# naver/deep-image-retrieval

Measured on AMD Instinct MI355X. Metric: images/sec descriptor extraction (resnet101-GeM, 1024x1024), higher is better.
Workload: dtype fp16p

## Files before the change

deep-image-retrieval_amd/csrc/conv_igemm.h:

```cpp
#pragma once
#include "dir_common.h"

namespace dir {

struct ConvArgs {
    const uint16_t* x;
    const uint16_t* w;
    const float* bias;
    const uint16_t* res;
    uint16_t* y;
    int B, H, W, Cin, OH, OW, Cout;
    int R, S, stride, pad, relu;
    int M;
    int Ktot;
    int T;
    int ksplit;
    float* partial;
    const uint16_t* w2;
    const float* bias2;
    uint16_t* y2;
    int Cout2, relu2;
    const uint16_t* x2;
    int Cin2;
    int H2, W2, stride2;
// ... 70 lines not shown
    a.T = a.Ktot / 64;
}
inline void conv_args_second_source(ConvArgs& a, const uint16_t* x2, const uint16_t* x2_lo, int Cin2) {
    a.x2 = x2;
    a.x2_lo = x2_lo;
    a.Cin2 = Cin2;
    a.Ktot = a.Cin + Cin2;
    a.T = a.Ktot / 64;
}
inline void conv_args_next_conv1(ConvArgs& a, const uint16_t* w2, const uint16_t* w2_lo, const float* bias2, uint16_t* y2,
                                 int Cout2, int relu2) {
    a.w2 = w2;
    a.w2_lo = w2_lo;
    a.bias2 = bias2;
    a.y2 = y2;
    a.Cout2 = Cout2;
    a.relu2 = relu2;
}

typedef bool (*ConvAdmissibleFn)(const ConvArgs&);
typedef hipError_t (*ConvLaunchFn)(const ConvArgs&, int dtype, hipStream_t);

struct ConvVariant {
    const char* name;
    int BM, BN, threads, stages, BK;
    ConvAdmissibleFn admissible;
    ConvLaunchFn launch;
    bool has_splitk;
    ConvAdmissibleFn admissible_dual;
    ConvLaunchFn launch_dual;
};

bool conv1x1_persist_admissible(const ConvArgs& a);
hipError_t conv1x1_persist_launch(const ConvArgs& a, int dtype, hipStream_t stream);
bool conv1x1_persist_x3_admissible(const ConvArgs& a);
hipError_t conv1x1_persist_x3_launch(const ConvArgs& a, int dtype, hipStream_t stream);
bool conv1x1_persist_dual_admissible(const ConvArgs& a);
hipError_t conv1x1_persist_dual_launch(const ConvArgs& a, int dtype, hipStream_t stream);
bool conv_patch64_lc_admissible(const ConvArgs& a);
hipError_t conv_patch64_lc_launch(const ConvArgs& a, int dtype, hipStream_t stream);
bool conv1x1_ring_admissible(const ConvArgs& a);
hipError_t conv1x1_ring_launch(const ConvArgs& a, int dtype, hipStream_t stream);
bool conv1x1_wreg_admissible(const ConvArgs& a);
hipError_t conv1x1_wreg_launch(const ConvArgs& a, int dtype, hipStream_t stream);
bool conv_small_admissible(const ConvArgs& a);
bool conv_small_k2_admissible(const ConvArgs& a);
hipError_t conv_small_s8_launch(const ConvArgs& a, int dtype, hipStream_t stream);
hipError_t conv_small_s4_launch(const ConvArgs& a, int dtype, hipStream_t stream);
hipError_t conv_small_s4k2_launch(const ConvArgs& a, int dtype, hipStream_t stream);
bool conv1x1_lc_admissible(const ConvArgs& a);
bool conv1x1_lc_plain_admissible(const ConvArgs& a);
hipError_t conv1x1_lc_launch(const ConvArgs& a, int dtype, hipStream_t stream);
hipError_t conv1x1_lc_dual_launch(const ConvArgs& a, int dtype, hipStream_t stream);
bool conv1x1_wregd_admissible(const ConvArgs& a);
hipError_t conv1x1_wregd_launch(const ConvArgs& a, int dtype, hipStream_t stream);
bool conv_seam3_admissible(const ConvArgs& a);
hipError_t conv_seam3_launch(const ConvArgs& a, int dtype, hipStream_t stream);
bool conv_c3c1_admissible(const ConvArgs& a);
bool conv_c3c1ds_lc_admissible(const ConvArgs& a);
hipError_t conv_c3c1ds_lc_launch(const ConvArgs& a, int dtype, hipStream_t stream);
hipError_t conv_c3c1_launch(const ConvArgs& a, int dtype, hipStream_t stream);
bool conv_patch3x3s_admissible(const ConvArgs& a);
hipError_t conv_patch3x3s_launch(const ConvArgs& a, int dtype, hipStream_t stream);
bool conv_patch3x3w_admissible(const ConvArgs& a);
hipError_t conv_patch3x3w_launch(const ConvArgs& a, int dtype, hipStream_t stream);
hipError_t conv_patch3x3w_pack(const uint16_t* w, uint16_t* out, int Cout, int Cin, hipStream_t stream);
bool conv_patch3x3s2_admissible(const ConvArgs& a);
hipError_t conv_patch3x3s2_launch(const ConvArgs& a, int dtype, hipStream_t stream);
hipError_t conv_patch3x3s2_pack(const uint16_t* w, uint16_t* out, int Cout, int Cin, hipStream_t stream);
bool conv_patch3x3_admissible(const ConvArgs& a);
hipError_t conv_patch3x3_launch(const ConvArgs& a, int dtype, hipStream_t stream);

int conv_pair_launch(const ConvArgs& a, hipStream_t stream);
const char* conv_pair_variant_name(const ConvArgs& a);

int conv_variant_count();
const ConvVariant& conv_variant(int i);
bool conv_variant_admissible(int v, const ConvArgs& a);
int conv_pick_variant(const ConvArgs& a);
int conv_pick_dual_variant(const ConvArgs& a, bool any_size = false);
int conv_launch(const ConvArgs& a, int dtype, int variant, hipStream_t stream);
int conv_splitk_factor(int v, const ConvArgs& a);
size_t conv_splitk_bytes(const ConvArgs& a, int ksplit);
constexpr size_t kSplitKMaxBytes = 64u << 20;
int conv_launch_naive(const ConvArgs& a, int dtype, hipStream_t stream);


}
```

deep-image-retrieval_amd/csrc/conv_persist.hip:

```cpp
#include "dir_common.h"
#include "conv_device.h"
#include "conv_igemm.h"

namespace dir {

template <class DT, bool XDEEP, bool RES, bool DUAL = false>
__global__ void __launch_bounds__(512) conv1x1_persist_kernel(const ConvArgs a) {
    static_assert(!DUAL || (XDEEP && !RES), "the two-source form rides on the deep-X ring");
    constexpr int BM = 256, BN = 256, NT = 512;
    constexpr int TM = 2, TN = 4;
    constexpr int NA = 4, NB = 4;
    constexpr int XS = BM * 128, STAGE = (BM + BN) * 128;
    constexpr int EROW = Staged<2>::EROW;
    constexpr int EPI_OFF = XDEEP ? XS : STAGE;
    constexpr int WOFF = 3 * XS;
    typedef typename DT::frag_t frag_t;

    extern __shared__ __attribute__((aligned(16))) char smem[];

    const int tid = threadIdx.x;
    const int lane = tid & 63;
    const int wave = __builtin_amdgcn_readfirstlane(tid >> 6);
    const int wn = wave & 1, wm = wave >> 1;
    const int lrow = lane & 31, lhi = lane >> 5;
    const int srcchunk = (tid & 7) ^ ((tid >> 4) & 7);

    const __amdgpu_buffer_rsrc_t rsrc_x = buffer_rsrc(a.x, a.x_bytes);
    const __amdgpu_buffer_rsrc_t rsrc_w = buffer_rsrc(a.w, a.w_bytes);
    const __amdgpu_buffer_rsrc_t rsrc_x2 = buffer_rsrc(DUAL ? a.x2 : a.x, DUAL ? a.x2_bytes : a.x_bytes);

    const int ntiles = a.tiles_m * a.tiles_n;
    const int T = a.T;
    const int T1 = DUAL ? a.Cin / 64 : 0;

    uint32_t xvoff[NA], wvoff[NB], xvoff2[DUAL ? NA : 1];
    auto tile_offsets = [&](int tile) {
        const int tile_n = tile % a.tiles_n, tile_m = a.rev_m ? a.tiles_m - 1 - tile / a.tiles_n : tile / a.tiles_n;
#pragma unroll
        for (int i = 0; i < NA; ++i) {
            const int m = tile_m * BM + i * 64 + (tid >> 3);
            uint32_t off;
            if (a.flat) {
#ifdef DIR_PERSIST_BLOCKED
                off = (uint32_t)(tile_m * (BM * a.Cin * 2) + (i * 64 + (tid >> 3)) * 128 + srcchunk * 16);
#else
                off = (uint32_t)((m * a.Cin + srcchunk * 8) * 2);
#endif
            } else {
                const uint32_t mm = m < a.M ? (uint32_t)m : 0u;
                const uint32_t b = fast_div(mm, a.div_ohw_mul, a.div_ohw_shr);
                const uint32_t rem = mm - b * (uint32_t)(a.OH * a.OW);
                const uint32_t oh = fast_div(rem, a.div_ow_mul, a.div_ow_shr);
                const uint32_t ow = rem - oh * (uint32_t)a.OW;
                off = (uint32_t)((((b * a.H + oh * a.stride) * a.W + ow * a.stride) * a.Cin +
                                  srcchunk * 8) * 2);
            }
            xvoff[i] = m < a.M ? off : kOOB;
            if (DUAL) {
                const uint32_t mm = m < a.M ? (uint32_t)m : 0u;
                const uint32_t b = fast_div(mm, a.div_ohw_mul, a.div_ohw_shr);
                const uint32_t rem = mm - b * (uint32_t)(a.OH * a.OW);
                const uint32_t oh = fast_div(rem, a.div_ow_mul, a.div_ow_shr);
                const uint32_t ow = rem - oh * (uint32_t)a.OW;
                const uint32_t off2 = (uint32_t)((((b * a.H2 + oh * a.stride2) * a.W2 + ow * a.stride2) * a.Cin2 +
                                                  srcchunk * 8) * 2);
                xvoff2[DUAL ? i : 0] = m < a.M ? off2 : kOOB;
            }
        }
#pragma unroll
        for (int i = 0; i < NB; ++i)
            wvoff[i] = (uint32_t)(((tile_n * BN + i * 64 + (tid >> 3)) * a.Ktot + srcchunk * 8) * 2);
    };
    auto issue_x = [&](int t, char* dst) {
        if (DUAL && t >= T1) {
#pragma unroll
            for (int i = 0; i < NA; ++i)
                dma16(rsrc_x2, dst + (i * NT + wave * 64) * 16, xvoff2[DUAL ? i : 0], (t - T1) * 128);
            return;
        }
#pragma unroll
#ifdef DIR_PERSIST_BLOCKED
        for (int i = 0; i < NA; ++i) dma16(rsrc_x, dst + (i * NT + wave * 64) * 16, xvoff[i], a.flat ? t * (BM * 128) : t * 128);
#else
        for (int i = 0; i < NA; ++i) dma16(rsrc_x, dst + (i * NT + wave * 64) * 16, xvoff[i], t * 128);
#endif
    };
    auto issue_w = [&](int t, char* dst) {
#pragma unroll
        for (int i = 0; i < NB; ++i) dma16(rsrc_w, dst + (i * NT + wave * 64) * 16, wvoff[i], t * 128);
    };
    auto issue = [&](int t, char* stage) {
        issue_x(t, stage);
        issue_w(t, stage + XS);
    };
    auto xslot = [&](int t) { return smem + (t % 3) * XS; };
    auto wslot = [&](int t) { return smem + WOFF + ((t + 1) & 1) * XS; };

    const int lswz = (lane >> 1) & 7;
    int loff[4];
#pragma unroll
    for (int ks = 0; ks < 4; ++ks) loff[ks] = lrow * 128 + (((2 * ks + lhi) ^ lswz) << 4);
    const int xfrag = (wm * TM * 32) * 128;
    const int wfrag = (XDEEP ? 0 : XS) + (wn * TN * 32) * 128;

    int tile = a.no_xcd_map ? (int)blockIdx.x : xcd_remap(blockIdx.x, gridDim.x);
    if (tile >= ntiles) return;
    Ovf<DT> ovf;
    f32x4_t bz[XDEEP ? TN : 1][XDEEP ? 4 : 1];
    auto load_bias = [&](int t) {
        if (!XDEEP) return;
        const int nw = (t % a.tiles_n) * BN + wn * TN * 32;
#pragma unroll
        for (int i = 0; i < TN; ++i)
#pragma unroll
            for (int g = 0; g < 4; ++g)
                bz[XDEEP ? i : 0][XDEEP ? g : 0] = bias4(a.bias + nw + i * 32, g, lhi);
    };
    load_bias(tile);
    tile_offsets(tile);
    if (XDEEP) {
        issue_w(0, wslot(0));
        issue_x(0, xslot(0));
        if (T > 1) issue_x(1, xslot(1));
    } else {
        issue(0, smem);
    }

    for (;;) {
        const int tile_n = tile % a.tiles_n, tile_m = a.rev_m ? a.tiles_m - 1 - tile / a.tiles_n : tile / a.tiles_n;
        const int m_epi = tile_m * BM + wm * TM * 32;
        const int n_wave = tile_n * BN + wn * TN * 32;

        f32x16_t acc[TN][TM];
        acc_init(acc, [&](int i, int g) {
            return XDEEP ? bz[XDEEP ? i : 0][XDEEP ? g : 0] : bias4(a.bias + n_wave + i * 32, g, lhi);
        });

        const int ecol = (lane & 7) * 8, erow = lane >> 3;
        u32x4_t rres[RES ? TM : 1][2][RES ? 4 : 1];
        if (RES && a.res) {
#pragma unroll
            for (int j = 0; j < TM; ++j)
#pragma unroll
                for (int h = 0; h < 2; ++h)
#pragma unroll
                    for (int pass = 0; pass < 4; ++pass) {
                        const int m = m_epi + j * 32 + pass * 8 + erow;
                        const int mc = m < a.M ? m : 0;
                        rres[RES ? j : 0][h][RES ? pass : 0] = gload16(a.res + ((size_t)mc * a.Cout + n_wave + h * 64 + ecol));
                    }
        }

        if (XDEEP) {
            for (int t = 0; t < T; ++t) {
                if (t + 1 < T && !(RES && t == 0 && a.res)) {
                    asm volatile("s_waitcnt vmcnt(%0)" ::"i"(NA) : "memory");
                } else {
                    asm volatile("s_waitcnt vmcnt(0)" ::: "memory");
                }
                ring_barrier();
                if (t + 1 < T) issue_w(t + 1, wslot(t + 1));
                if (t + 2 < T) issue_x(t + 2, xslot(t + 2));
                const char* xs = xslot(t);
                const char* ws = wslot(t);
#pragma unroll
                for (int ks = 0; ks < 4; ++ks) {
                    frag_t wf[TN], xf[TM];
#pragma unroll
                    for (int i = 0; i < TN; ++i) wf[i] = *(const frag_t*)(ws + wfrag + i * 4096 + loff[ks]);
#pragma unroll
                    for (int j = 0; j < TM; ++j) xf[j] = *(const frag_t*)(xs + xfrag + j * 4096 + loff[ks]);
#pragma unroll
                    for (int i = 0; i < TN; ++i)
#pragma unroll
                        for (int j = 0; j < TM; ++j) acc[i][j] = DT::mfma32(wf[i], xf[j], acc[i][j]);
                }
            }
        } else {
        int issued = 1;
        for (int t = 0; t < T; ++t) {
            asm volatile("s_waitcnt vmcnt(0)" ::: "memory");
            ring_barrier();
            if (issued < T) {
                issue(issued, smem + (issued & 1) * STAGE);
                ++issued;
            }
            const char* stage = smem + (t & 1) * STAGE;
#pragma unroll
            for (int ks = 0; ks < 4; ++ks) {
                frag_t wf[TN], xf[TM];
#pragma unroll
                for (int i = 0; i < TN; ++i) wf[i] = *(const frag_t*)(stage + wfrag + i * 4096 + loff[ks]);
#pragma unroll
                for (int j = 0; j < TM; ++j) xf[j] = *(const frag_t*)(stage + xfrag + j * 4096 + loff[ks]);
#pragma unroll
                for (int i = 0; i < TN; ++i)
#pragma unroll
                    for (int j = 0; j < TM; ++j) acc[i][j] = DT::mfma32(wf[i], xf[j], acc[i][j]);
            }
        }
        }
        __syncthreads();

        const int next = tile + (int)gridDim.x;
        if (next < ntiles) {
            load_bias(next);
            tile_offsets(next);
            if (XDEEP) {
                issue_w(0, wslot(0));
                issue_x(0, xslot(0));
            } else {
                issue(0, smem);
            }
        }

        char* ebase = smem + EPI_OFF + wave * (32 * EROW);
#pragma unroll
        for (int j = 0; j < TM; ++j)
#pragma unroll
            for (int h = 0; h < 2; ++h)
                epilogue_strip<2>(ebase, lrow, lhi, ecol, erow, [&](int ii) -> const f32x16_t& { return acc[2 * h + ii][j]; },
                                  [&](int pass, int mrow, float (&v)[8]) {
                    const int m = m_epi + j * 32 + mrow;
                    if (m < a.M) {
                        if (RES && a.res) add_res8<DT>(v, rres[RES ? j : 0][h][RES ? pass : 0]);
                        if (a.relu) relu8(v);
                        const u32x4_t ov = pack8<DT>(v);
                        gstore16(a.y + ((size_t)m * a.Cout + n_wave + h * 64 + ecol), ov);
                        ovf.see(ov);
                    }
                });
        if (next >= ntiles) break;
        if (XDEEP && T > 1) {
            asm volatile("s_waitcnt lgkmcnt(0)" ::: "memory");
            ring_barrier();
            issue_x(1, xslot(1));
        }
        tile = next;
    }
    ovf.flush(a.ovf);
}

bool conv1x1_persist_admissible(const ConvArgs& a) {
    return a.R == 1 && a.S == 1 && a.pad == 0 && a.Cout % 256 == 0 && a.Cin % 64 == 0 && a.Cin >= 128;
}

template <class DT, bool XDEEP, bool DUAL = false>
static hipError_t launch_persist(const ConvArgs& a, hipStream_t stream) {
    constexpr int LDS = XDEEP ? 5 * 256 * 128 : (256 + 256) * 128 + 8 * 32 * (2 * 128 + 16);
    static_assert(LDS >= 2 * (256 + 256) * 128 && LDS <= 160 * 1024, "LDS map");
    static_assert(!XDEEP || 256 * 128 + 8 * 32 * (2 * 128 + 16) <= 3 * 256 * 128 + 256 * 128, "staging must end below W slot 1");
    auto kern = conv1x1_persist_kernel<DT, XDEEP, !XDEEP, DUAL>;
    static std::atomic<uint64_t> attr_done{0};
    if (hipError_t e = ensure_dynamic_lds((const void*)kern, LDS, attr_done); e != hipSuccess) return e;
    ConvArgs b = a;
    b.T = a.Ktot / 64;
    b.tiles_m = ceil_div(a.M, 256);
    b.tiles_n = a.Cout / 256;
    conv_fill_extents(b);
    b.flat = (a.stride == 1 && a.H == a.OH && a.W == a.OW);
    const bool no_xcd_map = env().no_xcdmap;
    b.no_xcd_map = no_xcd_map;
    const int ntiles = b.tiles_m * b.tiles_n;
    const int ncu = cu_count();
    const int grid = ntiles < ncu ? ntiles : ncu;
    hipLaunchKernelGGL(kern, dim3(grid), dim3(512), LDS, stream, b);
    return hipGetLastError();
}

bool conv1x1_persist_dual_admissible(const ConvArgs& a) { return a.Cout % 256 == 0; }
hipError_t conv1x1_persist_dual_launch(const ConvArgs& a, int dtype, hipStream_t stream) {
    return dtype == DIR_BF16 ? launch_persist<BF16, true, true>(a, stream) : launch_persist<FP16, true, true>(a, stream);
}

bool conv1x1_persist_x3_admissible(const ConvArgs& a) { return conv1x1_persist_admissible(a) && a.res == nullptr; }
hipError_t conv1x1_persist_x3_launch(const ConvArgs& a, int dtype, hipStream_t stream) {
    return dtype == DIR_BF16 ? launch_persist<BF16, true>(a, stream) : launch_persist<FP16, true>(a, stream);
}

hipError_t conv1x1_persist_launch(const ConvArgs& a, int dtype, hipStream_t stream) {
    return dtype == DIR_BF16 ? launch_persist<BF16, false>(a, stream) : launch_persist<FP16, false>(a, stream);
}

}
```

deep-image-retrieval_amd/csrc/conv_persistlc.hip:

```cpp
#include "dir_common.h"
#include "conv_device.h"
#include "conv_igemm.h"

namespace dir {

template <class DT, bool DUAL>
__global__ void __launch_bounds__(768) conv1x1_lc_kernel(const ConvArgs a) {
    constexpr int BM = 256, BN = 256;
    constexpr int TM = 2, TN = 4;
    constexpr int XS = BM * 128;
    constexpr int WOFF = 3 * XS;
    constexpr int NL = 16;
    typedef typename DT::frag_t frag_t;

    extern __shared__ __attribute__((aligned(16))) char smem[];

    const int tid = threadIdx.x;
    const int lane = tid & 63;
    const int wave = __builtin_amdgcn_readfirstlane(tid >> 6);
    const int lrow = lane & 31, lhi = lane >> 5;

    const int ntiles = a.tiles_m * a.tiles_n;
    const int T = a.T;
    const int first = a.no_xcd_map ? (int)blockIdx.x : xcd_remap(blockIdx.x, gridDim.x);
// ... 130 lines not shown
                        const int m = m_wave + j * 32 + lrow;
                        if (m < a.M) {
                            gstore16(a.y + ((size_t)m * a.Cout + n_wave + i * 32 + h * 16 + lhi * 8), ov);
                            ovf.see(ov);
                        }
                    }
            }
            tile += (int)gridDim.x;
            t = 0;
        } else {
            ++t;
        }
        xslot = xslot + 1 == 3 ? 0 : xslot + 1;
        wslot ^= 1;
    }
    ovf.flush(a.ovf);
}

bool conv1x1_lc_admissible(const ConvArgs& a) {
    const bool base = a.R == 1 && a.S == 1 && a.pad == 0 && a.stride == 1 && a.H == a.OH && a.W == a.OW && a.Cout % 256 == 0 &&
                      a.Cin % 64 == 0 && a.res == nullptr && a.ksplit <= 1;
    if (a.x2) return base && a.Cin2 % 64 == 0 && a.Ktot == a.Cin + a.Cin2 && a.OW > 1;
    return base && a.Cin >= 128;
}

bool conv1x1_lc_plain_admissible(const ConvArgs& a) { return a.x2 == nullptr && conv1x1_lc_admissible(a); }

template <class DT, bool DUAL>
static hipError_t launch_lc(const ConvArgs& a, hipStream_t stream) {
    constexpr int LDS = 5 * 256 * 128;
    static_assert(LDS <= 160 * 1024, "LDS map");
    auto kern = conv1x1_lc_kernel<DT, DUAL>;
    static std::atomic<uint64_t> attr_done{0};
    if (hipError_t e = ensure_dynamic_lds((const void*)kern, LDS, attr_done); e != hipSuccess) return e;
    ConvArgs b = a;
    b.T = a.Ktot / 64;
    b.tiles_m = ceil_div(a.M, 256);
    b.tiles_n = a.Cout / 256;
    conv_fill_extents(b);
    b.no_xcd_map = env().no_xcdmap;
    const int ntiles = b.tiles_m * b.tiles_n;
    const int ncu = cu_count();
    hipLaunchKernelGGL(kern, dim3(ntiles < ncu ? ntiles : ncu), dim3(768), LDS, stream, b);
    return hipGetLastError();
}

hipError_t conv1x1_lc_launch(const ConvArgs& a, int dtype, hipStream_t stream) {
    return dtype == DIR_BF16 ? launch_lc<BF16, false>(a, stream) : launch_lc<FP16, false>(a, stream);
}
hipError_t conv1x1_lc_dual_launch(const ConvArgs& a, int dtype, hipStream_t stream) {
    return dtype == DIR_BF16 ? launch_lc<BF16, true>(a, stream) : launch_lc<FP16, true>(a, stream);
}

}
```

deep-image-retrieval_amd/csrc/dir_common.h:

```cpp
#pragma once
#include <hip/hip_runtime.h>
#include <stdint.h>
#include <string.h>
#include <atomic>
#include <string>

#include "../../include/dir_engine.h"

namespace dir {

typedef __attribute__((ext_vector_type(8))) __bf16 bf16x8_t;
typedef __attribute__((ext_vector_type(8))) _Float16 f16x8_t;
typedef __attribute__((ext_vector_type(16))) float f32x16_t;
typedef __attribute__((ext_vector_type(4))) float f32x4_t;
typedef __attribute__((ext_vector_type(4))) uint32_t u32x4_t;
typedef __attribute__((ext_vector_type(2))) uint32_t u32x2_t;
typedef __attribute__((ext_vector_type(4))) int i32x4_t;
typedef __attribute__((ext_vector_type(16))) int i32x16_t;
typedef __attribute__((ext_vector_type(2))) float f32x2_t;
typedef __attribute__((ext_vector_type(2))) __bf16 bf16x2_t;
typedef __attribute__((ext_vector_type(2))) _Float16 f16x2_t;

#define DIR_GLOBAL __attribute__((address_space(1)))
#define DIR_LDS __attribute__((address_space(3)))

void set_error(const std::string& msg);
int fail(int code, const std::string& msg);

#define DIR_HIP_CHECK(expr)                                                                \
    do {                                                                                   \
        hipError_t _e = (expr);                                                            \
        if (_e != hipSuccess)                                                              \
            return ::dir::fail(DIR_ERR_HIP, std::string(#expr) + ": " + hipGetErrorString(_e)); \
    } while (0)

#define DIR_CHECK(expr)                  \
    do {                                 \
        const int _rc = (expr);          \
        if (_rc != DIR_OK) return _rc;   \
    } while (0)

struct Env {
    bool c3c1_off = false, c3c1_force = false;
    bool no_ds_seam = false, no_dual = false;
    bool rev_conv1 = false, rev_conv3 = false;
    bool unfused_stem = false, stem_v1 = false;
    bool no_patchlc = false, no_wreg = false, no_patchw = false, no_x3 = false, no_patchs = false;
    bool patchw_pack = false, no_patchw_pack = false;
    bool small_k2 = false;
    bool no_patchs2 = false;
    bool x3_k2048 = false;
    bool lc1x1 = false;
    bool no_c3c1lc = false;
    bool no_smallmap = false;
    bool no_wregd = false;
    bool no_patchw_lc = false;
    bool no_xcdmap = false;
    bool no_pair_patch = false, pair_acts = false;
    int pair_stages = 1;
    bool sim_v1 = false, sim_exact = false;
    bool experiments = false;
    bool no_inplace = false;
    bool seam_full_store = false;
    bool no_stem_u8 = false;
    bool stem_pair_old = false;
    bool stem_u8_prep = false;
    bool stem_u8_wg8 = false;
    int stem_u8_seg = 0;
};
const Env& env();
void reload_env();

__host__ __device__ inline uint16_t f32_to_bf16_bits(float f) {
    uint32_t u;
    memcpy(&u, &f, 4);
    if ((u & 0x7fffffffu) > 0x7f800000u) return (uint16_t)((u >> 16) | 0x40);
    u += 0x7fffu + ((u >> 16) & 1u);
    return (uint16_t)(u >> 16);
}
__host__ __device__ inline float bf16_bits_to_f32(uint16_t h) {
    uint32_t u = ((uint32_t)h) << 16;
    float f;
    memcpy(&f, &u, 4);
    return f;
}
__host__ __device__ inline uint16_t f32_to_f16_bits(float f) {
    _Float16 h = (_Float16)f;
    uint16_t b;
    memcpy(&b, &h, 2);
    return b;
}
__host__ __device__ inline float f16_bits_to_f32(uint16_t b) {
    _Float16 h;
    memcpy(&h, &b, 2);
    return (float)h;
}

struct BF16 {
    typedef bf16x8_t frag_t;
    static constexpr int kDtype = DIR_BF16;
    __host__ __device__ static inline float to_f32(uint16_t b) { return bf16_bits_to_f32(b); }
    __host__ __device__ static inline uint16_t from_f32(float f) { return f32_to_bf16_bits(f); }
    __device__ static inline f32x16_t mfma32(frag_t a, frag_t b, f32x16_t c) {
        return __builtin_amdgcn_mfma_f32_32x32x16_bf16(a, b, c, 0, 0, 0);
    }
    __device__ static inline void unpack(uint32_t w, float& lo, float& hi) {
        lo = __builtin_bit_cast(float, w << 16);
        hi = __builtin_bit_cast(float, w & 0xffff0000u);
    }
    __device__ static inline uint32_t pack(float lo, float hi) {
// ... 121 lines not shown
```

deep-image-retrieval_amd/csrc/engine.hip:

```cpp
#include "engine.h"

#include <math.h>
#include <algorithm>

namespace dir {

static thread_local std::string g_err;
void set_error(const std::string& msg) { g_err = msg; }
int fail(int code, const std::string& msg) {
    g_err = msg;
    return code;
}
const char* last_error() { return g_err.c_str(); }


static Env read_env() {
    Env e;
    auto on = [](const char* k) { return getenv(k) != nullptr; };
    const char* mode = getenv("DIRTORCH_AMD_C3C1");
    e.c3c1_off = mode && mode[0] == '0';
    e.c3c1_force = mode && mode[0] == 'f';
    e.no_ds_seam = on("DIRTORCH_AMD_NO_DS_SEAM");
    e.no_dual = on("DIRTORCH_AMD_NO_DUAL");
    e.rev_conv1 = on("DIRTORCH_AMD_REV_CONV1");
    e.rev_conv3 = on("DIRTORCH_AMD_REV_CONV3");
    e.unfused_stem = on("DIRTORCH_AMD_UNFUSED_STEM");
    e.stem_v1 = on("DIRTORCH_AMD_STEM_V1");
    e.no_patchlc = on("DIRTORCH_AMD_NO_PATCHLC");
    e.no_wreg = on("DIRTORCH_AMD_NO_WREG");
    e.no_wregd = on("DIRTORCH_AMD_NO_WREGD");
    e.no_smallmap = on("DIRTORCH_AMD_NO_SMALLMAP");
    e.no_c3c1lc = on("DIRTORCH_AMD_NO_C3C1LC");
    e.lc1x1 = on("DIRTORCH_AMD_LC1X1");
    e.x3_k2048 = on("DIRTORCH_AMD_X3_K2048");
    e.no_patchs2 = on("DIRTORCH_AMD_NO_PATCHS2");
    e.small_k2 = on("DIRTORCH_AMD_SMALL_K2");
    e.patchw_pack = on("DIRTORCH_AMD_PATCHW_PACK");
    e.no_patchw_pack = on("DIRTORCH_AMD_NO_PATCHW_PACK");
    e.no_patchw = on("DIRTORCH_AMD_NO_PATCHW");
    e.no_x3 = on("DIRTORCH_AMD_NO_X3");
    e.no_patchs = on("DIRTORCH_AMD_NO_PATCHS");
    e.no_patchw_lc = on("DIRTORCH_AMD_NO_PATCHW_LC");
    e.no_xcdmap = on("DIRTORCH_AMD_NO_XCDMAP");
    e.no_pair_patch = on("DIRTORCH_AMD_NO_PAIR_PATCH");
    e.pair_acts = on("DIRTORCH_AMD_PAIR_ACTS");
    if (const char* s = getenv("DIRTORCH_AMD_PAIR_STAGES")) e.pair_stages = atoi(s);
    e.sim_v1 = on("DIRTORCH_AMD_SIM_V1");
    e.sim_exact = on("DIRTORCH_AMD_SIM_EXACT");
    e.experiments = on("DIRTORCH_AMD_EXPERIMENTS");
    e.no_inplace = on("DIRTORCH_AMD_NO_INPLACE");
    e.seam_full_store = on("DIRTORCH_AMD_SEAM_FULL_STORE");
    e.no_stem_u8 = on("DIRTORCH_AMD_NO_STEM_U8");
    e.stem_u8_wg8 = on("DIRTORCH_AMD_STEM_U8_WG8");
    e.stem_u8_prep = on("DIRTORCH_AMD_STEM_U8_PREP");
    e.stem_pair_old = on("DIRTORCH_AMD_STEM_PAIR_OLD");
    if (const char* s = getenv("DIRTORCH_AMD_STEM_U8_SEG")) e.stem_u8_seg = atoi(s);
    return e;
}
static Env g_env[2];
static std::atomic<int> g_env_cur{-1};
static std::atomic_flag g_env_lock = ATOMIC_FLAG_INIT;
static void publish_env() {
    while (g_env_lock.test_and_set(std::memory_order_acquire)) {
    }
    const int cur = g_env_cur.load(std::memory_order_relaxed);
    const int nxt = cur < 0 ? 0 : 1 - cur;
    g_env[nxt] = read_env();
    g_env_cur.store(nxt, std::memory_order_release);
    g_env_lock.clear(std::memory_order_release);
}
const Env& env() {
    int cur = g_env_cur.load(std::memory_order_acquire);
    if (cur < 0) {
        static const bool once = (publish_env(), true);
        (void)once;
        cur = g_env_cur.load(std::memory_order_acquire);
    }
    return g_env[cur];
}
void reload_env() { publish_env(); }

static inline size_t align_up(size_t v, size_t a = 256) { return (v + a - 1) / a * a; }

__global__ void fill_noise_kernel(uint16_t* p, long n, int dtype) {
    const long i = (long)blockIdx.x * blockDim.x + threadIdx.x;
    if (i >= n) return;
    uint32_t h = (uint32_t)i * 2654435761u + 12345u;
    h ^= h >> 15;
    h *= 2246822519u;
    h ^= h >> 13;
    const float f = (float)(h & 0xffff) / 32768.f - 1.f;
    p[i] = dtype == DIR_BF16 ? f32_to_bf16_bits(f) : f32_to_f16_bits(f);
}

}

// ... 907 lines not shown
```

deep-image-retrieval_amd/csrc/conv_device.h:

```cpp
#pragma once
#include "dir_common.h"

namespace dir {

static constexpr uint32_t kOOB = 0x80000000u;

__device__ __forceinline__ __amdgpu_buffer_rsrc_t buffer_rsrc(const void* ptr, uint32_t bytes) {
    return __builtin_amdgcn_make_buffer_rsrc((void*)ptr, 0, bytes, 0x00020000);
}

__device__ __forceinline__ void dma16(__amdgpu_buffer_rsrc_t rsrc, char* lds, uint32_t voff, int soff) {
    __builtin_amdgcn_raw_ptr_buffer_load_lds(rsrc, (DIR_LDS void*)lds, 16, voff, soff, 0, 0);
}

__device__ __forceinline__ void bstore16(__amdgpu_buffer_rsrc_t rsrc, uint32_t voff, int soff, u32x4_t v) {
    __builtin_amdgcn_raw_buffer_store_b128(v, rsrc, voff, soff, 0);
}

__device__ __forceinline__ uint32_t fast_div(uint32_t n, uint32_t mul, uint32_t shr) {
    return mul ? (__umulhi(n, mul) >> shr) : n;
}

__device__ __forceinline__ void wave_lds_sync() {
    __builtin_amdgcn_fence(__ATOMIC_RELEASE, "wavefront");
    __builtin_amdgcn_wave_barrier();
    __builtin_amdgcn_fence(__ATOMIC_ACQUIRE, "wavefront");
}

template <bool CIN16 = false, class A>
__device__ __forceinline__ void im2col_lane(const A& a, int m, int chunk, int& xbase, uint32_t& xmask) {
    const bool mvalid = m < a.M;
    const uint32_t mm = mvalid ? (uint32_t)m : 0u;
    const uint32_t b = fast_div(mm, a.div_ohw_mul, a.div_ohw_shr);
    const uint32_t rem = mm - b * (uint32_t)(a.OH * a.OW);
    const uint32_t oh = fast_div(rem, a.div_ow_mul, a.div_ow_shr);
    const uint32_t ow = rem - oh * (uint32_t)a.OW;
    const int ih0 = (int)oh * a.stride - a.pad;
    const int iw0 = (int)ow * a.stride - a.pad;
    xbase = (((int)b * a.H + ih0) * a.W + iw0) * a.Cin * 2 + chunk * 16;
    auto range_bits = [](int lo, int hi) -> uint32_t { return hi > lo ? (((1u << hi) - 1u) & ~((1u << lo) - 1u)) : 0u; };
    const uint32_t rbits = range_bits(max(0, -ih0), min(CIN16 ? 4 : a.R, a.H - ih0));
    if (CIN16) {
        const bool wok = (unsigned)(iw0 + (chunk >> 1)) < (unsigned)a.W;
        xmask = (mvalid && wok) ? rbits : 0u;
    } else {
        const uint32_t cbits = range_bits(max(0, -iw0), min(a.S, a.W - iw0));
        uint32_t mask = 0;
#pragma unroll
        for (int r = 0; r < 4; ++r) mask |= ((rbits >> r) & 1u) ? (cbits << (r * a.S)) : 0u;
        xmask = mvalid ? mask : 0u;
    }
}

template <int BK, bool CIN16 = false>
struct KWalker {
    int tap = 0, cc = 0, r = 0, s = 0;
    template <class A>
    __device__ __forceinline__ void seek(const A& a, int t) {
        if (CIN16) {
            r = tap = t;
        } else {
            const int taps = a.R * a.S;
            cc = t / taps;
            tap = t - cc * taps;
            r = tap / a.S;
            s = tap - r * a.S;
        }
    }
    template <class A>
// ... 165 lines not shown
```

Measured before the change: 2520.

## Add warp-specialized persistent 1x1 conv kernel overlapping epilogue stores with MFMA

Adds a persistent 1x1 conv kernel in which four dedicated waves stream X and W tiles into a three-slot LDS ring, while eight compute waves process each 256x256 tile as two 128-wide halves. Storing the previous half's accumulators is interleaved with the first k-steps of the next half, so epilogue writes are hidden behind matrix math. The persist launchers route two-source convolutions with deep K to this kernel unless an env flag disables it. This costs more registers, since two accumulator sets are held, and a narrower per-wave tile.

Measured after the change: 2517 (median of 2 runs). No clear change (-0.1%).

```diff
diff --git a/deep-image-retrieval_amd/csrc/conv_igemm.h b/deep-image-retrieval_amd/csrc/conv_igemm.h
--- a/deep-image-retrieval_amd/csrc/conv_igemm.h
+++ b/deep-image-retrieval_amd/csrc/conv_igemm.h
@@ -146,6 +146,8 @@
 bool conv1x1_lc_plain_admissible(const ConvArgs& a);
 hipError_t conv1x1_lc_launch(const ConvArgs& a, int dtype, hipStream_t stream);
 hipError_t conv1x1_lc_dual_launch(const ConvArgs& a, int dtype, hipStream_t stream);
+bool conv1x1_overlap_admissible(const ConvArgs& a);
+hipError_t conv1x1_overlap_launch(const ConvArgs& a, int dtype, hipStream_t stream);
 bool conv1x1_wregd_admissible(const ConvArgs& a);
 hipError_t conv1x1_wregd_launch(const ConvArgs& a, int dtype, hipStream_t stream);
 bool conv_seam3_admissible(const ConvArgs& a);
diff --git a/deep-image-retrieval_amd/csrc/conv_persist.hip b/deep-image-retrieval_amd/csrc/conv_persist.hip
--- a/deep-image-retrieval_amd/csrc/conv_persist.hip
+++ b/deep-image-retrieval_amd/csrc/conv_persist.hip
@@ -268,17 +268,25 @@
     return hipGetLastError();
 }
 
+static bool persist_overlap_pays(const ConvArgs& a) {
+    if (env().no_persist_overlap || !conv1x1_overlap_admissible(a)) return false;
+    return a.x2 != nullptr && a.Ktot / 64 >= 16;
+}
+
 bool conv1x1_persist_dual_admissible(const ConvArgs& a) { return a.Cout % 256 == 0; }
 hipError_t conv1x1_persist_dual_launch(const ConvArgs& a, int dtype, hipStream_t stream) {
+    if (persist_overlap_pays(a)) return conv1x1_overlap_launch(a, dtype, stream);
     return dtype == DIR_BF16 ? launch_persist<BF16, true, true>(a, stream) : launch_persist<FP16, true, true>(a, stream);
 }
 
 bool conv1x1_persist_x3_admissible(const ConvArgs& a) { return conv1x1_persist_admissible(a) && a.res == nullptr; }
 hipError_t conv1x1_persist_x3_launch(const ConvArgs& a, int dtype, hipStream_t stream) {
+    if (persist_overlap_pays(a)) return conv1x1_overlap_launch(a, dtype, stream);
     return dtype == DIR_BF16 ? launch_persist<BF16, true>(a, stream) : launch_persist<FP16, true>(a, stream);
 }
 
 hipError_t conv1x1_persist_launch(const ConvArgs& a, int dtype, hipStream_t stream) {
+    if (persist_overlap_pays(a)) return conv1x1_overlap_launch(a, dtype, stream);
     return dtype == DIR_BF16 ? launch_persist<BF16, false>(a, stream) : launch_persist<FP16, false>(a, stream);
 }
 
diff --git a/deep-image-retrieval_amd/csrc/conv_persistlc.hip b/deep-image-retrieval_amd/csrc/conv_persistlc.hip
--- a/deep-image-retrieval_amd/csrc/conv_persistlc.hip
+++ b/deep-image-retrieval_amd/csrc/conv_persistlc.hip
@@ -206,4 +206,227 @@
     return dtype == DIR_BF16 ? launch_lc<BF16, true>(a, stream) : launch_lc<FP16, true>(a, stream);
 }
 
-}
+template <class DT, bool DUAL>
+__global__ void __launch_bounds__(768) conv1x1_overlap_kernel(const ConvArgs a) {
+    constexpr int BM = 256, BN = 256, HN = 128;
+    constexpr int TM = 2, TN = 2;
+    constexpr int XS = BM * 128, WS = HN * 128;
+    constexpr int WOFF = 3 * XS;
+    constexpr int BIAS_OFF = WOFF + 3 * WS;
+    constexpr int NLX = 8, NLW = 4;
+    typedef typename DT::frag_t frag_t;
+
+    extern __shared__ __attribute__((aligned(16))) char smem[];
+
+    const int tid = threadIdx.x;
+    const int lane = tid & 63;
+    const int wave = __builtin_amdgcn_readfirstlane(tid >> 6);
+    const int lrow = lane & 31, lhi = lane >> 5;
+
+    const int ntiles = a.tiles_m * a.tiles_n;
+    const int T = a.T;
+    const int first = a.no_xcd_map ? (int)blockIdx.x : xcd_remap(blockIdx.x, gridDim.x);
+    if (first >= ntiles) return;
+    const int my_tiles = (ntiles - first + (int)gridDim.x - 1) / (int)gridDim.x;
+    const int total = my_tiles * 2 * T;
+
+    if (wave >= 8) {
+        const int part = wave - 8;
+        const int T1 = DUAL ? a.Cin / 64 : T;
+        const __amdgpu_buffer_rsrc_t rsrc_x = buffer_rsrc(a.x, a.x_bytes);
+        const __amdgpu_buffer_rsrc_t rsrc_w = buffer_rsrc(a.w, a.w_bytes);
+        const __amdgpu_buffer_rsrc_t rsrc_x2 = buffer_rsrc(DUAL ? a.x2 : a.x, DUAL ? a.x2_bytes : a.x_bytes);
+        const int rsub = lane >> 3;
+        const int chE = (lane & 7) ^ (lane >> 4), chO = (lane & 7) ^ (4 + (lane >> 4));
+        const uint32_t xstride = (uint32_t)(8 * a.Cin * 2), wstride = (uint32_t)(8 * a.Ktot * 2);
+        uint32_t xE = 0, xO = 0, wE = 0, wO = 0;
+        uint32_t voff2[NLX];
+        int m0 = 0;
+        auto unit_offsets = [&](int u) __attribute__((always_inline)) {
+            const int tile = first + (u >> 1) * (int)gridDim.x;
+            const int tile_n = tile % a.tiles_n, tile_m = a.rev_m ? a.tiles_m - 1 - tile / a.tiles_n : tile / a.tiles_n;
+            m0 = tile_m * BM + part * (NLX * 8) + rsub;
+            xE = (uint32_t)((m0 * a.Cin + chE * 8) * 2);
+            xO = (uint32_t)((m0 * a.Cin + chO * 8) * 2);
+            if constexpr (DUAL) {
+#pragma unroll
+                for (int k = 0; k < NLX; ++k) {
+                    const int m = m0 + 8 * k;
+                    const uint32_t mm = m < a.M ? (uint32_t)m : 0u;
+                    const uint32_t b = fast_div(mm, a.div_ohw_mul, a.div_ohw_shr);
+                    const uint32_t rem = mm - b * (uint32_t)(a.OH * a.OW);
+                    const uint32_t oh = fast_div(rem, a.div_ow_mul, a.div_ow_shr);
+                    const uint32_t ow = rem - oh * (uint32_t)a.OW;
+                    const uint32_t off2 = (((b * a.H2 + oh * a.stride2) * a.W2 + ow * a.stride2) * a.Cin2 + ((k & 1) ? chO : chE) * 8) * 2;
+                    voff2[k] = m < a.M ? off2 : kOOB;
+                }
+            }
+            const int r0 = tile_n * BN + (u & 1) * HN + part * (NLW * 8) + rsub;
+            wE = (uint32_t)((r0 * a.Ktot + chE * 8) * 2);
+            wO = (uint32_t)((r0 * a.Ktot + chO * 8) * 2);
+        };
+        int is_u = 0, is_t = 0, is_slot = 0;
+        unit_offsets(0);
+        auto issue_next = [&]() __attribute__((always_inline)) {
+            char* xdst = smem + is_slot * XS + part * (NLX * 1024);
+            char* wdst = smem + WOFF + is_slot * WS + part * (NLW * 1024);
+            bool second = false;
+            if constexpr (DUAL) second = is_t >= T1;
+            if (second) {
+                if constexpr (DUAL) {
+#pragma unroll
+                    for (int k = 0; k < NLX; ++k) dma16(rsrc_x2, xdst + k * 1024, voff2[k], (is_t - T1) * 128);
+                }
+            } else {
+#pragma unroll
+                for (int k2 = 0; k2 < NLX / 2; ++k2) {
+                    const uint32_t offe = m0 + 16 * k2 < a.M ? xE + (uint32_t)(2 * k2) * xstride : kOOB;
+                    dma16(rsrc_x, xdst + (2 * k2) * 1024, offe, is_t * 128);
+                    const uint32_t offo = m0 + 16 * k2 + 8 < a.M ? xO + (uint32_t)(2 * k2 + 1) * xstride : kOOB;
+                    dma16(rsrc_x, xdst + (2 * k2 + 1) * 1024, offo, is_t * 128);
+                }
+            }
+#pragma unroll
+            for (int k2 = 0; k2 < NLW / 2; ++k2) {
+                dma16(rsrc_w, wdst + (2 * k2) * 1024, wE + (uint32_t)(2 * k2) * wstride, is_t * 128);
+                dma16(rsrc_w, wdst + (2 * k2 + 1) * 1024, wO + (uint32_t)(2 * k2 + 1) * wstride, is_t * 128);
+            }
+            is_slot = is_slot + 1 == 3 ? 0 : is_slot + 1;
+            if (++is_t == T) {
+                is_t = 0;
+                if (++is_u < 2 * my_tiles) unit_offsets(is_u);
+            }
+        };
+        issue_next();
+        issue_next();
+        ring_barrier();
+        for (int g = 0; g < total; ++g) {
+            if (g + 1 < total) {
+                asm volatile("s_waitcnt vmcnt(%0)" ::"i"(NLX + NLW) : "memory");
+            } else {
+                asm volatile("s_waitcnt vmcnt(0)" ::: "memory");
+            }
+            ring_barrier();
+            if (g + 2 < total) issue_next();
+        }
+        return;
+    }
+
+    const int wn = wave & 1, wm = wave >> 1;
+    const int lswz = (lane >> 1) & 7;
+    int loff[4];
+#pragma unroll
+    for (int ks = 0; ks < 4; ++ks) loff[ks] = lrow * 128 + (((2 * ks + lhi) ^ lswz) << 4);
+    const int xfrag = (wm * TM * 32) * 128;
+    const int wfrag = WOFF + (wn * TN * 32) * 128;
+    float* const sbias = (float*)(smem + BIAS_OFF);
+    for (int i = tid; i < a.Cout / 4; i += 512) ((f32x4_t*)sbias)[i] = *(const DIR_GLOBAL f32x4_t*)(a.bias + 4 * i);
+    asm volatile("s_waitcnt lgkmcnt(0)" ::: "memory");
+    ring_barrier();
+
+    const uint32_t y_bytes = (uint32_t)a.M * (uint32_t)a.Cout * 2u;
+    const __amdgpu_buffer_rsrc_t rsrc_y = buffer_rsrc(a.y, y_bytes);
+    const int jstep = 32 * a.Cout * 2;
+    Ovf<DT> ovf;
+    f32x16_t accA[TN][TM], accB[TN][TM];
+    acc_init_zero(accB);
+    uint32_t dvoff[TM] = {kOOB, kOOB};
+    int slot = 0;
+
+    auto drain2 = [&](f32x16_t (&prv)[TN][TM], int q) __attribute__((always_inline)) {
+        const int i = q >> 1, j = q & 1;
+        const bool ok = dvoff[j] != kOOB;
+#pragma unroll
+        for (int h = 0; h < 2; ++h) {
+            const u32x4_t ov = swap_pack16<DT>(prv[i][j], h, a.relu);
+            bstore16(rsrc_y, dvoff[j], j * jstep + i * 64 + h * 32, ov);
+#pragma unroll
+            for (int e = 0; e < 4; ++e) ovf.see(ok ? ov[e] : 0u);
+        }
+    };
+    auto kstep = [&](f32x16_t (&cur)[TN][TM]) __attribute__((always_inline)) {
+        const char* xs = smem + slot * XS;
+        const char* ws = smem + slot * WS;
+#pragma unroll
+        for (int ks = 0; ks < 4; ++ks) {
+            frag_t wf[TN], xf[TM];
+#pragma unroll
+            for (int i = 0; i < TN; ++i) wf[i] = *(const frag_t*)(ws + wfrag + i * 4096 + loff[ks]);
+#pragma unroll
+            for (int j = 0; j < TM; ++j) xf[j] = *(const frag_t*)(xs + xfrag + j * 4096 + loff[ks]);
+#pragma unroll
+            for (int j = 0; j < TM; ++j)
+#pragma unroll
+                for (int i = 0; i < TN; ++i) cur[i][j] = DT::mfma32(wf[i], xf[j], cur[i][j]);
+        }
+        asm volatile("s_waitcnt lgkmcnt(0)" ::: "memory");
+        slot = slot + 1 == 3 ? 0 : slot + 1;
+    };
+    auto half_tile = [&](f32x16_t (&cur)[TN][TM], f32x16_t (&prv)[TN][TM], int tile, int half) __attribute__((always_inline)) {
+        const int tile_n = tile % a.tiles_n, tile_m = a.rev_m ? a.tiles_m - 1 - tile / a.tiles_n : tile / a.tiles_n;
+        const int n_wave = tile_n * BN + half * HN + wn * TN * 32;
+        const int m_lane = tile_m * BM + wm * TM * 32 + lrow;
+        const uint32_t yoff = (uint32_t)((m_lane * a.Cout + n_wave + lhi * 8) * 2);
+        acc_init(cur, [&](int i, int g) { return bias4<true>(sbias + n_wave + i * 32, g, lhi); });
+        int t = 0;
+#pragma unroll
+        for (int q = 0; q < 4; ++q) {
+            if (t < T) {
+                ring_barrier();
+                drain2(prv, q);
+                kstep(cur);
+                ++t;
+            } else {
+                drain2(prv, q);
+            }
+        }
+        for (; t < T; ++t) {
+            ring_barrier();
+            kstep(cur);
+        }
+#pragma unroll
+        for (int j = 0; j < TM; ++j) dvoff[j] = m_lane + 32 * j < a.M ? yoff : kOOB;
+    };
+
+    for (int tile = first; tile < ntiles; tile += (int)gridDim.x) {
+        half_tile(accA, accB, tile, 0);
+        half_tile(accB, accA, tile, 1);
+    }
+#pragma unroll
+    for (int q = 0; q < 4; ++q) drain2(accB, q);
+    ovf.flush(a.ovf);
+}
+
+bool conv1x1_overlap_admissible(const ConvArgs& a) {
+    const bool base = a.R == 1 && a.S == 1 && a.pad == 0 && a.stride == 1 && a.H == a.OH && a.W == a.OW && a.Cout % 256 == 0 &&
+                      a.Cout <= 4096 && a.Cin % 64 == 0 && a.ksplit <= 1 && a.res == nullptr &&
+                      ((size_t)a.M + 256) * a.Cout * 2 < (1ull << 31);
+    if (a.x2) return base && a.Cin2 % 64 == 0 && a.Ktot == a.Cin + a.Cin2;
+    return base && a.Cin >= 128;
+}
+
+template <class DT, bool DUAL>
+static hipError_t launch_overlap(const ConvArgs& a, hipStream_t stream) {
+    constexpr int LDS = 3 * (256 + 128) * 128 + 4096 * 4;
+    static_assert(LDS <= 160 * 1024, "LDS map");
+    auto kern = conv1x1_overlap_kernel<DT, DUAL>;
+    static std::atomic<uint64_t> attr_done{0};
+    if (hipError_t e = ensure_dynamic_lds((const void*)kern, LDS, attr_done); e != hipSuccess) return e;
+    ConvArgs b = a;
+    b.T = a.Ktot / 64;
+    b.tiles_m = ceil_div(a.M, 256);
+    b.tiles_n = a.Cout / 256;
+    conv_fill_extents(b);
+    b.no_xcd_map = env().no_xcdmap;
+    const int ntiles = b.tiles_m * b.tiles_n;
+    const int ncu = cu_count();
+    hipLaunchKernelGGL(kern, dim3(ntiles < ncu ? ntiles : ncu), dim3(768), LDS, stream, b);
+    return hipGetLastError();
+}
+
+hipError_t conv1x1_overlap_launch(const ConvArgs& a, int dtype, hipStream_t stream) {
+    if (a.x2) return dtype == DIR_BF16 ? launch_overlap<BF16, true>(a, stream) : launch_overlap<FP16, true>(a, stream);
+    return dtype == DIR_BF16 ? launch_overlap<BF16, false>(a, stream) : launch_overlap<FP16, false>(a, stream);
+}
+
+}
diff --git a/deep-image-retrieval_amd/csrc/dir_common.h b/deep-image-retrieval_amd/csrc/dir_common.h
--- a/deep-image-retrieval_amd/csrc/dir_common.h
+++ b/deep-image-retrieval_amd/csrc/dir_common.h
@@ -56,6 +56,7 @@
     bool no_wregd = false;
     bool no_patchw_lc = false;
     bool no_xcdmap = false;
+    bool no_persist_overlap = false;
     bool no_pair_patch = false, pair_acts = false;
     int pair_stages = 1;
     bool sim_v1 = false, sim_exact = false;
diff --git a/deep-image-retrieval_amd/csrc/engine.hip b/deep-image-retrieval_amd/csrc/engine.hip
--- a/deep-image-retrieval_amd/csrc/engine.hip
+++ b/deep-image-retrieval_amd/csrc/engine.hip
@@ -42,6 +42,7 @@
     e.no_patchs = on("DIRTORCH_AMD_NO_PATCHS");
     e.no_patchw_lc = on("DIRTORCH_AMD_NO_PATCHW_LC");
     e.no_xcdmap = on("DIRTORCH_AMD_NO_XCDMAP");
+    e.no_persist_overlap = on("DIRTORCH_AMD_NO_PERSIST_OVERLAP");
     e.no_pair_patch = on("DIRTORCH_AMD_NO_PAIR_PATCH");
     e.pair_acts = on("DIRTORCH_AMD_PAIR_ACTS");
     if (const char* s = getenv("DIRTORCH_AMD_PAIR_STAGES")) e.pair_stages = atoi(s);
```

## Store persistent 1x1 conv epilogue directly from registers, skipping LDS staging

Applied to the files above, without the earlier changes.

Adds compile-time modes to the persistent 1x1 conv kernel. In the default XDEEP path the output tile is written straight from MFMA accumulators with buffer stores (swap_pack16) instead of being staged through LDS. Residual values are preloaded into registers in the accumulator layout, the accumulators are re-initialised early, and the next tile's X prefetch is issued before the epilogue. The waitcnt accounting is adjusted for the outstanding stores. This is meant to remove the LDS round trip and wave syncs in the epilogue and to overlap the next tile's loads. In exchange it raises register pressure and relies on hand-tuned vmcnt values.

New measurement: 2510 before, 2497 after. Within noise of the previous version (-0.5%).

```diff
diff --git a/deep-image-retrieval_amd/csrc/conv_device.h b/deep-image-retrieval_amd/csrc/conv_device.h
--- a/deep-image-retrieval_amd/csrc/conv_device.h
+++ b/deep-image-retrieval_amd/csrc/conv_device.h
@@ -15,6 +15,15 @@
 
 __device__ __forceinline__ void bstore16(__amdgpu_buffer_rsrc_t rsrc, uint32_t voff, int soff, u32x4_t v) {
     __builtin_amdgcn_raw_buffer_store_b128(v, rsrc, voff, soff, 0);
+}
+
+__device__ __forceinline__ void bstore16_hold(__amdgpu_buffer_rsrc_t rsrc, uint32_t voff, u32x4_t v) {
+    __builtin_amdgcn_raw_buffer_store_b128(v, rsrc, voff, 0, 0);
+    asm volatile("s_nop 1" ::"v"(v) : "memory");
+}
+
+__device__ __forceinline__ u32x2_t bload8(__amdgpu_buffer_rsrc_t rsrc, uint32_t voff, int soff) {
+    return __builtin_amdgcn_raw_buffer_load_b64(rsrc, voff, soff, 0);
 }
 
 __device__ __forceinline__ uint32_t fast_div(uint32_t n, uint32_t mul, uint32_t shr) {
diff --git a/deep-image-retrieval_amd/csrc/conv_persist.hip b/deep-image-retrieval_amd/csrc/conv_persist.hip
--- a/deep-image-retrieval_amd/csrc/conv_persist.hip
+++ b/deep-image-retrieval_amd/csrc/conv_persist.hip
@@ -1,8 +1,19 @@
+#ifndef DIR_PERSIST_STAGED
+#define DIR_PERSIST_STAGED 0
+#endif
+#ifndef DIR_PERSIST_2SLOT_STAGED
+#define DIR_PERSIST_2SLOT_STAGED 1
+#endif
+#include <type_traits>
+
 #include "dir_common.h"
 #include "conv_device.h"
 #include "conv_igemm.h"
 
 namespace dir {
+
+constexpr int persist_mode(bool XDEEP, bool , bool ) { return XDEEP ? DIR_PERSIST_STAGED : (DIR_PERSIST_STAGED != 0 || DIR_PERSIST_2SLOT_STAGED); }
+constexpr bool persist_staged(bool XDEEP, bool RES, bool DUAL) { return persist_mode(XDEEP, RES, DUAL) == 1 || persist_mode(XDEEP, RES, DUAL) == 2; }
 
 template <class DT, bool XDEEP, bool RES, bool DUAL = false>
 __global__ void __launch_bounds__(512) conv1x1_persist_kernel(const ConvArgs a) {
@@ -11,9 +22,12 @@
     constexpr int TM = 2, TN = 4;
     constexpr int NA = 4, NB = 4;
     constexpr int XS = BM * 128, STAGE = (BM + BN) * 128;
+    constexpr int MODE = persist_mode(XDEEP, RES, DUAL);
+    constexpr bool STAGED = persist_staged(XDEEP, RES, DUAL);
     constexpr int EROW = Staged<2>::EROW;
-    constexpr int EPI_OFF = XDEEP ? XS : STAGE;
+    constexpr int EPI_OFF = XDEEP ? (MODE >= 2 ? 2 * XS : XS) : STAGE;
     constexpr int WOFF = 3 * XS;
+    constexpr int NST = TN * TM * 2;
     typedef typename DT::frag_t frag_t;
 
     extern __shared__ __attribute__((aligned(16))) char smem[];
@@ -28,6 +42,9 @@
     const __amdgpu_buffer_rsrc_t rsrc_x = buffer_rsrc(a.x, a.x_bytes);
     const __amdgpu_buffer_rsrc_t rsrc_w = buffer_rsrc(a.w, a.w_bytes);
     const __amdgpu_buffer_rsrc_t rsrc_x2 = buffer_rsrc(DUAL ? a.x2 : a.x, DUAL ? a.x2_bytes : a.x_bytes);
+    const uint32_t y_bytes = (uint32_t)a.M * (uint32_t)a.Cout * 2u;
+    const __amdgpu_buffer_rsrc_t rsrc_y = buffer_rsrc(a.y, y_bytes);
+    const __amdgpu_buffer_rsrc_t rsrc_r = buffer_rsrc(RES && a.res ? (const void*)a.res : (const void*)a.y, y_bytes);
 
     const int ntiles = a.tiles_m * a.tiles_n;
     const int T = a.T;
@@ -125,35 +142,63 @@
     } else {
         issue(0, smem);
     }
+    bool primed = false;
+
+    constexpr bool EARLY_ACC = XDEEP && !STAGED;
+    f32x16_t acc[TN][TM];
+    auto acc_from_bz = [&]() { acc_init(acc, [&](int i, int g) { return bz[XDEEP ? i : 0][XDEEP ? g : 0]; }); };
+    if constexpr (EARLY_ACC) acc_from_bz();
 
     for (;;) {
         const int tile_n = tile % a.tiles_n, tile_m = a.rev_m ? a.tiles_m - 1 - tile / a.tiles_n : tile / a.tiles_n;
         const int m_epi = tile_m * BM + wm * TM * 32;
         const int n_wave = tile_n * BN + wn * TN * 32;
 
-        f32x16_t acc[TN][TM];
-        acc_init(acc, [&](int i, int g) {
-            return XDEEP ? bz[XDEEP ? i : 0][XDEEP ? g : 0] : bias4(a.bias + n_wave + i * 32, g, lhi);
-        });
+        if constexpr (!EARLY_ACC) {
+            acc_init(acc, [&](int i, int g) {
+                return XDEEP ? bz[XDEEP ? i : 0][XDEEP ? g : 0] : bias4(a.bias + n_wave + i * 32, g, lhi);
+            });
+        }
 
         const int ecol = (lane & 7) * 8, erow = lane >> 3;
-        u32x4_t rres[RES ? TM : 1][2][RES ? 4 : 1];
-        if (RES && a.res) {
-#pragma unroll
-            for (int j = 0; j < TM; ++j)
-#pragma unroll
-                for (int h = 0; h < 2; ++h)
-#pragma unroll
-                    for (int pass = 0; pass < 4; ++pass) {
-                        const int m = m_epi + j * 32 + pass * 8 + erow;
-                        const int mc = m < a.M ? m : 0;
-                        rres[RES ? j : 0][h][RES ? pass : 0] = gload16(a.res + ((size_t)mc * a.Cout + n_wave + h * 64 + ecol));
-                    }
+        constexpr bool RS = RES && STAGED, RR = RES && !STAGED;
+        u32x4_t rres[RS ? TM : 1][2][RS ? 4 : 1];
+        u32x2_t rreg[RR ? TN : 1][RR ? TM : 1][RR ? 4 : 1];
+        if constexpr (RR) {
+            if (a.res) {
+#pragma unroll
+                for (int j = 0; j < TM; ++j) {
+                    const int m = m_epi + j * 32 + lrow;
+                    const uint32_t row = m < a.M ? (uint32_t)m * (uint32_t)(a.Cout * 2) + (uint32_t)((n_wave + 4 * lhi) * 2) : kOOB;
+#pragma unroll
+                    for (int i = 0; i < TN; ++i)
+#pragma unroll
+                        for (int g = 0; g < 4; ++g) rreg[i][j][g] = bload8(rsrc_r, row, (i * 32 + 8 * g) * 2);
+                }
+            }
+        }
+        if constexpr (RS) {
+            if (a.res) {
+#pragma unroll
+                for (int j = 0; j < TM; ++j)
+#pragma unroll
+                    for (int h = 0; h < 2; ++h)
+#pragma unroll
+                        for (int pass = 0; pass < 4; ++pass) {
+                            const int m = m_epi + j * 32 + pass * 8 + erow;
+                            const int mc = m < a.M ? m : 0;
+                            rres[j][h][pass] = gload16(a.res + ((size_t)mc * a.Cout + n_wave + h * 64 + ecol));
+                        }
+            }
         }
 
         if (XDEEP) {
             for (int t = 0; t < T; ++t) {
-                if (t + 1 < T && !(RES && t == 0 && a.res)) {
+                if (MODE == 2 && primed && t == 0) {
+                    asm volatile("s_waitcnt vmcnt(0)" ::: "memory");
+                } else if (!STAGED && primed && t == 0 && t + 1 < T && !(RES && a.res)) {
+                    asm volatile("s_waitcnt vmcnt(%0)" ::"i"(NA + NST) : "memory");
+                } else if (t + 1 < T && !(RES && t == 0 && a.res)) {
                     asm volatile("s_waitcnt vmcnt(%0)" ::"i"(NA) : "memory");
                 } else {
                     asm volatile("s_waitcnt vmcnt(0)" ::: "memory");
@@ -207,34 +252,107 @@
             load_bias(next);
             tile_offsets(next);
             if (XDEEP) {
-                issue_w(0, wslot(0));
+                if (MODE != 2) issue_w(0, wslot(0));
                 issue_x(0, xslot(0));
+                if (MODE != 1 && T > 1) issue_x(1, xslot(1));
             } else {
                 issue(0, smem);
             }
         }
 
-        char* ebase = smem + EPI_OFF + wave * (32 * EROW);
-#pragma unroll
-        for (int j = 0; j < TM; ++j)
-#pragma unroll
-            for (int h = 0; h < 2; ++h)
-                epilogue_strip<2>(ebase, lrow, lhi, ecol, erow, [&](int ii) -> const f32x16_t& { return acc[2 * h + ii][j]; },
-                                  [&](int pass, int mrow, float (&v)[8]) {
-                    const int m = m_epi + j * 32 + mrow;
-                    if (m < a.M) {
-                        if (RES && a.res) add_res8<DT>(v, rres[RES ? j : 0][h][RES ? pass : 0]);
-                        if (a.relu) relu8(v);
-                        const u32x4_t ov = pack8<DT>(v);
-                        gstore16(a.y + ((size_t)m * a.Cout + n_wave + h * 64 + ecol), ov);
-                        ovf.see(ov);
+        if constexpr (!STAGED) {
+            __builtin_amdgcn_sched_barrier(0);
+            if constexpr (MODE == 3) {
+                typedef Staged<1> G1;
+                char* ebase1 = smem + EPI_OFF + wave * (32 * G1::EROW);
+                const int ecol1 = (lane & 3) * 8, erow1 = lane >> 2;
+#pragma unroll
+                for (int j = 0; j < TM; ++j)
+#pragma unroll
+                    for (int i = 0; i < TN; ++i)
+                        epilogue_strip<1>(ebase1, lrow, lhi, ecol1, erow1, [&](int) -> const f32x16_t& { return acc[i][j]; },
+                                          [&](int, int mrow, float (&v)[8]) {
+                            const int m = m_epi + j * 32 + mrow;
+                            const bool mok = m < a.M;
+                            if (a.relu) relu8(v);
+                            const u32x4_t ov = pack8<DT>(v);
+                            bstore16_hold(rsrc_y, mok ? (uint32_t)m * (uint32_t)(a.Cout * 2) + (uint32_t)((n_wave + i * 32 + ecol1) * 2) : kOOB, ov);
+                            ovf.see(mok ? ov : u32x4_t{0u, 0u, 0u, 0u});
+                        });
+            }
+            auto store_tile = [&](auto has_res) {
+#pragma unroll
+                for (int j = 0; j < TM; ++j) {
+                    const int m = m_epi + j * 32 + lrow;
+                    const bool mok = m < a.M;
+                    const uint32_t row = mok ? (uint32_t)m * (uint32_t)(a.Cout * 2) + (uint32_t)((n_wave + 8 * lhi) * 2) : kOOB;
+#pragma unroll
+                    for (int i = 0; i < TN; ++i) {
+                        f32x4_t add[4];
+                        if constexpr (decltype(has_res)::value) {
+#pragma unroll
+                            for (int g = 0; g < 4; ++g) {
+                                float r0, r1, r2, r3;
+                                DT::unpack(rreg[i][j][g][0], r0, r1);
+                                DT::unpack(rreg[i][j][g][1], r2, r3);
+                                add[g] = f32x4_t{r0, r1, r2, r3};
+                            }
+                        }
+#pragma unroll
+                        for (int h = 0; h < 2; ++h) {
+                            u32x4_t ov;
+                            if constexpr (decltype(has_res)::value)
+                                ov = swap_pack16<DT>(acc[i][j], h, a.relu, add);
+                            else
+                                ov = swap_pack16<DT>(acc[i][j], h, a.relu);
+                            bstore16_hold(rsrc_y, row + (uint32_t)((i * 32 + h * 16) * 2), ov);
+                            ovf.see(mok ? ov : u32x4_t{0u, 0u, 0u, 0u});
+                        }
                     }
-                });
-        if (next >= ntiles) break;
-        if (XDEEP && T > 1) {
-            asm volatile("s_waitcnt lgkmcnt(0)" ::: "memory");
-            ring_barrier();
-            issue_x(1, xslot(1));
+                }
+            };
+            if constexpr (RR) {
+                if (a.res)
+                    store_tile(std::true_type{});
+                else
+                    store_tile(std::false_type{});
+            } else if constexpr (MODE != 3) {
+                store_tile(std::false_type{});
+            }
+            __builtin_amdgcn_sched_barrier(0);
+            if (next >= ntiles) break;
+            primed = true;
+            if constexpr (EARLY_ACC) acc_from_bz();
+        } else {
+            char* ebase = smem + EPI_OFF + wave * (32 * EROW);
+#pragma unroll
+            for (int j = 0; j < TM; ++j)
+#pragma unroll
+                for (int h = 0; h < 2; ++h)
+                    epilogue_strip<2>(ebase, lrow, lhi, ecol, erow, [&](int ii) -> const f32x16_t& { return acc[2 * h + ii][j]; },
+                                      [&](int pass, int mrow, float (&v)[8]) {
+                        const int m = m_epi + j * 32 + mrow;
+                        if (m < a.M) {
+                            if constexpr (RS) {
+                                if (a.res) add_res8<DT>(v, rres[j][h][pass]);
+                            }
+                            if (a.relu) relu8(v);
+                            const u32x4_t ov = pack8<DT>(v);
+                            gstore16(a.y + ((size_t)m * a.Cout + n_wave + h * 64 + ecol), ov);
+                            ovf.see(ov);
+                        }
+                    });
+            if (next >= ntiles) break;
+            if (XDEEP && T > 1) {
+                asm volatile("s_waitcnt lgkmcnt(0)" ::: "memory");
+                ring_barrier();
+                if (MODE == 2) {
+                    issue_w(0, wslot(0));
+                    primed = true;
+                } else {
+                    issue_x(1, xslot(1));
+                }
+            }
         }
         tile = next;
     }
@@ -247,9 +365,11 @@
 
 template <class DT, bool XDEEP, bool DUAL = false>
 static hipError_t launch_persist(const ConvArgs& a, hipStream_t stream) {
-    constexpr int LDS = XDEEP ? 5 * 256 * 128 : (256 + 256) * 128 + 8 * 32 * (2 * 128 + 16);
+    constexpr bool STAGED = persist_staged(XDEEP, !XDEEP, DUAL);
+    constexpr int STAGING = 8 * 32 * Staged<2>::EROW;
+    constexpr int LDS = XDEEP ? 5 * 256 * 128 : STAGED ? (256 + 256) * 128 + STAGING : 2 * (256 + 256) * 128;
     static_assert(LDS >= 2 * (256 + 256) * 128 && LDS <= 160 * 1024, "LDS map");
-    static_assert(!XDEEP || 256 * 128 + 8 * 32 * (2 * 128 + 16) <= 3 * 256 * 128 + 256 * 128, "staging must end below W slot 1");
+    static_assert(!STAGED || !XDEEP || 2 * 256 * 128 + STAGING <= 160 * 1024, "staging must fit");
     auto kern = conv1x1_persist_kernel<DT, XDEEP, !XDEEP, DUAL>;
     static std::atomic<uint64_t> attr_done{0};
     if (hipError_t e = ensure_dynamic_lds((const void*)kern, LDS, attr_done); e != hipSuccess) return e;
```
